# td-kwj-zp2023/webgpu-msm-bls12-377

Measured on AMD Instinct MI355X. Metric: ms per 2^20 BLS12-377 G1 MSM, lower is better.
Workload: dtype u32 (29-bit limbs, 64-bit accumulate)

## Files before the change

### webgpu-msm-bls12-377_amd/csrc/capi.hip

```cpp
#include <hip/hip_runtime.h>
#include <stdlib.h>
#include <string.h>

#include <algorithm>
#include <new>

#include "context.hpp"
#include "host_tail.hpp"
#include "sequencer.hpp"
#include "import_host.hpp"
#include "validate_host.hpp"

using namespace msm377;

#define HIP_TRY(ctx, call)                                                  \
  do {                                                                      \
    if (!eng::hip_ok((ctx), (int)(call), #call)) return MSM377_EHIP;        \
  } while (0)


extern "C" {

const char* msm377_version(void) { return "msm377 0.1 gfx950"; }

const char* msm377_strerror(int code) {
  switch (code) {
    case MSM377_OK: return "ok";
    case MSM377_EINVAL: return "invalid argument";
    case MSM377_EHIP: return "HIP runtime error";
    case MSM377_ESCALAR: return "scalar out of range for the signed window recode";
    case MSM377_ENOMEM: return "out of memory";
    case MSM377_ESTATE: return "call sequence error";
    case MSM377_EGLVRANGE: return "scalar outside the GLV range";
    case MSM377_EEXCEPTIONAL: return "exceptional case of the twisted Edwards law while combining partial records";
    case MSM377_EPOINT: return "an input point failed a requested check (canonical / on the curve / in the subgroup)";
    default: return "unknown error";
  }
}

int msm377_ctx_create(int device, uint64_t max_points, msm377_ctx** out) {
  if (!out || max_points == 0 || max_points > (1ull << 30)) return MSM377_EINVAL;
  *out = nullptr;
  int count = 0;
  if (hipGetDeviceCount(&count) != hipSuccess || device < 0 || device >= count) return MSM377_EHIP;
  msm377_ctx* ctx = new (std::nothrow) msm377_ctx();
  if (!ctx) return MSM377_ENOMEM;
  ctx->device = device;
  ctx->cap = max_points;
  if (const char* e = getenv("MSM377_GLV")) ctx->glv_mode = atoi(e);
  if (const char* e = getenv("MSM377_G1_FORM")) ctx->g1_form = atoi(e) != 0;
  if (const char* e = getenv("MSM377_CONV_WAVE_PRIO")) ctx->conv_wave_prio = atoi(e) != 0;
  if (const char* e = getenv("MSM377_AFF_PREWAKE_US")) ctx->aff_prewake_us = atoll(e);
  if (const char* e = getenv("MSM377_UPLOAD_CHUNKS")) ctx->upload_chunks = (uint32_t)std::min(std::max(atoi(e), 2), 7);
  if (const char* e = getenv("MSM377_UPLOAD_SPLIT")) ctx->upload_split_pct = (uint32_t)std::min(std::max(atoi(e), 5), 90);
  if (const char* e = getenv("MSM377_UPLOAD_CHUNK_MIN")) ctx->upload_chunk_min = strtoull(e, nullptr, 10);
  if (const char* e = getenv("MSM377_TAIL_THREADS")) ctx->tail_threads = std::min(std::max(atoi(e), 1), TailPool::WORKERS + 1);
  if (const char* e = getenv("MSM377_TAIL_WAIT_MS")) ctx->tail_pool.wait_limit_ns = (int64_t)std::max(atoi(e), 1) * 1000000ll;
  if (const char* e = getenv("MSM377_TAIL_SPIN_US")) ctx->tail_spin_us = atoll(e);
  if (const char* e = getenv("MSM377_TAIL_TRACE")) ctx->tail_trace = atoi(e) != 0;
  if (const char* e = getenv("MSM377_TAIL_NUMA")) ctx->tail_pool.numa_local = atoi(e) != 0;
  if (const char* e = getenv("MSM377_TE_AFFINE_MSM")) ctx->te_affine_msm = atoi(e) != 0;
  if (const char* e = getenv("MSM377_NARROW_MAX")) ctx->narrow_max_points = strtoull(e, nullptr, 10);
  if (const char* e = getenv("MSM377_PRECOMP_BITS")) ctx->precomp_bits = atoi(e) == (int)WIDE_BITS ? (int)WIDE_BITS : MSM377_WINDOW_BITS;
  if (const char* e = getenv("MSM377_AFFINE_MIN")) ctx->affine_min_points = strtoull(e, nullptr, 10);
  if (const char* e = getenv("MSM377_SEG_PLAIN")) ctx->seg_plain = std::min(std::max(atoi(e), (int)SEG_MIN), (int)SEG_MAX);
  if (const char* e = getenv("MSM377_SEG_GLV")) ctx->seg_glv = std::min(std::max(atoi(e), (int)SEG_MIN), (int)SEG_MAX);
  if (const char* e = getenv("MSM377_ZERO_COPY_OUT")) ctx->zc_out = atoi(e);
  if (const char* e = getenv("MSM377_NARROW_SEG")) ctx->narrow_seg = (uint32_t)std::min(std::max(atoi(e), (int)NARROW_SEG), (int)SEG_BINS - 1);
  if (const char* e = getenv("MSM377_NARROW_QUAD_ITEMS")) ctx->narrow_quad_items = strtoull(e, nullptr, 10);
  if (const char* e = getenv("MSM377_COOP_THREADS")) ctx->coop_threads = (uint32_t)atoi(e);
  if (const char* e = getenv("MSM377_NARROW_TAIL_FROM")) ctx->narrow_tail_from = (uint32_t)std::min(std::max(atoi(e), 1), (int)TREE_LEVELS);
  if (const char* e = getenv("MSM377_TAIL_LDS")) ctx->tail_lds = atoi(e) != 0;
  if (const char* e = getenv("MSM377_EVEN_WINDOWS")) ctx->even_windows = atoi(e) != 0;
  if (const char* e = getenv("MSM377_TWIN_BATCH")) ctx->twin_batches = atoi(e) != 0;
  if (const char* e = getenv("MSM377_BASE_CHECKS")) ctx->base_checks = check_flags_normal((uint32_t)strtoul(e, nullptr, 0));
  if (const char* e = getenv("MSM377_TAIL_FROM")) ctx->tail_from = (uint32_t)std::min(std::max(atoi(e), 1), (int)TREE_LEVELS);
  const uint64_t cap = max_points;
  int prio_least = 0, prio_greatest = 0;
  bool ok = hipSetDevice(device) == hipSuccess;
  if (ok && hipDeviceGetStreamPriorityRange(&prio_least, &prio_greatest) != hipSuccess) prio_least = prio_greatest = 0;
  ok = ok && hipStreamCreateWithPriority(&ctx->stream, hipStreamNonBlocking, prio_greatest) == hipSuccess &&
            hipStreamCreateWithPriority(&ctx->stream2, hipStreamNonBlocking, prio_least) == hipSuccess &&
            hipEventCreateWithFlags(&ctx->bases_ready, hipEventDisableTiming) == hipSuccess;
  auto dalloc = [&](void** p, size_t bytes) { ok = ok && hipMalloc(p, bytes) == hipSuccess; };
  dalloc((void**)&ctx->d_raw_points, cap * 96);
  dalloc((void**)&ctx->d_raw_scalars, cap * 32);
  dalloc((void**)&ctx->d_bases, 2 * cap * G1_REC_WORDS * 4);
  const uint64_t wcap = std::max<uint64_t>((uint64_t)MSM377_NUM_WINDOWS * cap, (uint64_t)NARROW_EVEN_WINDOWS * std::min<uint64_t>(cap, SMALL_SORT_MAX));
  dalloc((void**)&ctx->d_digits, wcap * 2);
  dalloc((void**)&ctx->d_range_counts, (size_t)NRANGE * MAX_SORT_BLOCKS * 4);
  dalloc((void**)&ctx->d_region_base, (size_t)MSM377_NUM_WINDOWS * (NRANGE + 1) * 4);
  dalloc((void**)&ctx->d_sort_temp, cap * MSM377_NUM_WINDOWS * sizeof(SortElem));
  dalloc((void**)&ctx->d_row_ptr, (size_t)MSM377_NUM_WINDOWS * RP * 4);
  dalloc((void**)&ctx->d_val_idx, wcap * 4);
  dalloc((void**)&ctx->d_buckets, (size_t)MSM377_NUM_WINDOWS * BKT_WORDS * NB * 4);
  dalloc((void**)&ctx->d_partials, (size_t)2 * SLOT_WORDS * 4);
  const uint64_t extra_items = std::max<uint64_t>((uint64_t)MSM377_NUM_WINDOWS * cap / SEG_MIN, (uint64_t)NARROW_EVEN_WINDOWS * std::min<uint64_t>(cap, SMALL_SORT_MAX) / NARROW_SEG) + 2;
  dalloc((void**)&ctx->d_work, ((size_t)MSM377_NUM_WINDOWS * NB + extra_items) * sizeof(WorkItem));
  dalloc((void**)&ctx->d_work_meta, (size_t)META_BLOCK_WORDS * 4);
  dalloc((void**)&ctx->d_row_ovf_base, (size_t)MSM377_NUM_WINDOWS * NB * 4);
  dalloc((void**)&ctx->d_split_rows, (size_t)MSM377_NUM_WINDOWS * NB * 4);
  dalloc((void**)&ctx->d_ovf, (size_t)extra_items * BKT_WORDS * 4);
  const size_t aff_blocks = (size_t)affine_blocks(cap) + 1;
  dalloc((void**)&ctx->d_aff_count, 64);
  ok = ok && hipMemset(ctx->d_aff_count, 0, 64) == hipSuccess;
  dalloc((void**)&ctx->d_aff_stash, (size_t)affine_blocks(cap) * AFF_BLOCK_POINTS * AFF_STASH_WORDS * 4);
  dalloc((void**)&ctx->d_aff_trees, aff_blocks * 2 * AFF_THREADS * 13 * 4);
  const unsigned host_flags = hipHostMallocMapped | hipHostMallocCoherent;
  ok = ok && hipHostMalloc((void**)&ctx->h_aff_prod, aff_blocks * 48, host_flags) == hipSuccess &&
       hipHostMalloc((void**)&ctx->h_aff_inv, aff_blocks * 48, host_flags) == hipSuccess &&
       hipHostMalloc((void**)&ctx->h_aff_flag, 64, host_flags) == hipSuccess &&
       hipHostGetDevicePointer((void**)&ctx->dm_aff_prod, ctx->h_aff_prod, 0) == hipSuccess &&
       hipHostGetDevicePointer((void**)&ctx->dm_aff_inv, ctx->h_aff_inv, 0) == hipSuccess &&
       hipHostGetDevicePointer((void**)&ctx->dm_aff_flag, ctx->h_aff_flag, 0) == hipSuccess &&
       hipEventCreateWithFlags(&ctx->aff_up_done, hipEventDisableTiming) == hipSuccess;
  if (ok) ctx->aff_scratch.resize(aff_blocks);
  dalloc((void**)&ctx->d_err, 4 * sizeof(int));
  ok = ok && hipHostMalloc((void**)&ctx->h_partials, (size_t)2 * SLOT_WORDS * 4, host_flags) == hipSuccess &&
       hipHostGetDevicePointer((void**)&ctx->dm_partials, ctx->h_partials, 0) == hipSuccess &&
       hipHostMalloc((void**)&ctx->h_out_flag, 64, host_flags) == hipSuccess &&
       hipHostGetDevicePointer((void**)&ctx->dm_out_flag, ctx->h_out_flag, 0) == hipSuccess;
  if (ok) memset(ctx->h_out_flag, 0, 64);
  dalloc((void**)&ctx->d_out_count, 64);
  ok = ok && hipMemset(ctx->d_out_count, 0, 64) == hipSuccess;
  ok = ok && hipHostMalloc((void**)&ctx->h_err, 2 * sizeof(int)) == hipSuccess;
  for (int k = 0; ok && k < 2; k++) ok = ok && hipEventCreateWithFlags(&ctx->done_ev[k], hipEventDisableTiming) == hipSuccess;
  for (int s = 0; ok && s < MSM377_NUM_STAGES; s++)
    for (int k = 0; k < 2; k++) ok = ok && hipEventCreate(&ctx->ev[s][k]) == hipSuccess;
  if (!ok) {
    msm377_ctx_destroy(ctx);
    return MSM377_ENOMEM;
  }
  *out = ctx;
  return MSM377_OK;
}

void msm377_ctx_destroy(msm377_ctx* ctx) {
  if (!ctx) return;
  ctx->tail_pool.shutdown();
  (void)hipSetDevice(ctx->device);
  if (ctx->stream) (void)hipStreamSynchronize(ctx->stream);
  if (ctx->stream2) (void)hipStreamSynchronize(ctx->stream2);
  if (ctx->twin) {
    eng::twin_return(ctx);
    msm377_ctx_destroy(ctx->twin);
    ctx->twin = nullptr;
  }
  void* bufs[] = {ctx->d_raw_points, ctx->d_raw_scalars, ctx->d_bases, ctx->d_digits, ctx->d_range_counts, ctx->d_region_base, ctx->d_sort_temp,
// ... 312 lines not shown
```

### webgpu-msm-bls12-377_amd/csrc/common.hpp

```cpp
#pragma once
#include <stdint.h>

#include "../../include/msm377.h"

namespace msm377 {

constexpr uint32_t NB = 32768;
constexpr uint32_t NBIN = NB + 1;
constexpr uint32_t RP = NBIN + 1;
constexpr uint32_t PT_WORDS = 52;
constexpr uint32_t BKT_WORDS = 64;
constexpr uint32_t MAX_SORT_BLOCKS = 256;
constexpr uint32_t TREE_LEVELS = 15;
constexpr uint32_t SEG_MIN = 16;
constexpr uint32_t SEG_MAX = 128;
constexpr uint32_t SEG_BINS = SEG_MAX + 1;
constexpr int ERR_SCALAR = 1, ERR_GLV_RANGE = 2, ERR_NARROW_RANGE = 128;
constexpr int ERR_SHORT_WIDTH = 256;
constexpr int ERR_TE_EXCEPTIONAL = MSM377_FB_ACCUMULATE, ERR_TE_MERGE = MSM377_FB_MERGE, ERR_TE_TREE = MSM377_FB_TREE, ERR_TE_CONVERT = MSM377_FB_CONVERT;
constexpr int ERR_TE_ANY = ERR_TE_EXCEPTIONAL | ERR_TE_MERGE | ERR_TE_TREE | ERR_TE_CONVERT;
constexpr uint32_t NARROW_LOG = 11;
constexpr uint32_t NARROW_SEG = 8;
constexpr uint32_t NARROW_EVEN_WINDOWS = 22, NARROW_EVEN_SIGNED = 11, NARROW_EVEN_BITS = NARROW_LOG + 1;
static_assert(NARROW_EVEN_SIGNED * NARROW_EVEN_BITS + (NARROW_EVEN_WINDOWS - NARROW_EVEN_SIGNED) * NARROW_LOG == 253, "the windows cover a 253-bit scalar");
constexpr uint32_t MAX_WINDOW_SLOTS = NARROW_EVEN_WINDOWS > MSM377_NUM_WINDOWS ? NARROW_EVEN_WINDOWS : MSM377_NUM_WINDOWS;

constexpr uint32_t short_windows(uint32_t bits, uint32_t L) { return bits / (L + 1) + 1; }
static_assert(short_windows(253, 15) == MSM377_NUM_WINDOWS && short_windows(253, NARROW_LOG) == NARROW_EVEN_WINDOWS, "at full width: the window counts of the main and the narrow path");

constexpr uint32_t NRANGE = 256;
constexpr uint32_t KRANGE = NB / NRANGE;
constexpr uint32_t KEY_TRACKED = 0x80000000u;
constexpr uint32_t KEY_UNSIGNED = 0x40000000u;
constexpr uint32_t SMALL_SORT_MAX = 1u << 16;
constexpr uint32_t SMALL_BINS_MAX = (1u << 12) + 1;
struct SortElem {
  uint32_t idx_sign;
  uint32_t key;
};

struct WorkItem {
  uint32_t row;
  uint32_t seg;
};
constexpr uint32_t META_BLOCK_WORDS = 2 * SEG_BINS + 4 + MSM377_NUM_WINDOWS;
constexpr size_t SLOT_WORDS = (size_t)MAX_WINDOW_SLOTS * MSM377_G1_PARTIAL_POINTS * MSM377_G1_POINT_WORDS;

constexpr uint32_t AFF_THREADS = 256, AFF_K = 8, AFF_BLOCK_POINTS = AFF_THREADS * AFF_K;
constexpr uint32_t AFF_STASH_WORDS = 52;
inline uint32_t affine_blocks(uint64_t n) { return (uint32_t)((n + AFF_BLOCK_POINTS - 1) / AFF_BLOCK_POINTS); }

constexpr uint32_t ACC_FLAG_WORD = 4;
constexpr uint32_t EVEN_FROM = 13;
constexpr uint32_t even_offset(uint32_t w) { return 16 * w - (w > EVEN_FROM ? w - EVEN_FROM : 0u); }
static_assert(even_offset(13) == 208 && even_offset(14) == 223 && even_offset(15) == 238 && even_offset(16) == 253, "13 x 16 + 3 x 15 = 253 bits");
constexpr uint32_t WIDE_BITS = MSM377_WIDE_WINDOW_BITS;
constexpr uint32_t WIDE_LOG = 19;
constexpr uint32_t WIDE_WINDOWS = 13;
constexpr uint32_t WIDE_FULL = 6;
constexpr uint32_t wide_width(uint32_t w) { return w < WIDE_FULL ? WIDE_BITS : WIDE_BITS - 1; }
constexpr uint32_t wide_offset(uint32_t w) { return w <= WIDE_FULL ? WIDE_BITS * w : WIDE_BITS * WIDE_FULL + (WIDE_BITS - 1) * (w - WIDE_FULL); }
static_assert(wide_offset(WIDE_WINDOWS - 1) == 234 && wide_offset(WIDE_WINDOWS - 1) + wide_width(WIDE_WINDOWS - 1) == 253, "the windows cover a 253-bit scalar");
constexpr uint32_t WIDE_NRANGE = 4096;
constexpr uint32_t WIDE_POINTS = WIDE_LOG + 1;
static_assert((1u << WIDE_LOG) == WIDE_NRANGE * KRANGE, "ranges of KRANGE keys cover the wide bucket set");
static_assert((1u << WIDE_LOG) <= MSM377_NUM_WINDOWS * NB, "the wide bucket set fits the main path's bucket, row and work-list buffers");
static_assert(WIDE_POINTS * 1 <= MAX_WINDOW_SLOTS * MSM377_G1_PARTIAL_POINTS, "the wide window record fits a partial-record slot");

constexpr uint32_t G1_REC_WORDS = 32;
constexpr uint32_t GLV_WINDOWS = MSM377_GLV_WINDOWS;

}
```

### webgpu-msm-bls12-377_amd/csrc/context.hpp

```cpp
#pragma once
#include <hip/hip_runtime.h>

#include <functional>
#include <string>
#include <vector>

#include "common.hpp"
#include "fp64_host.hpp"
#include "tail_pool.hpp"

using msm377::SortElem;
using msm377::WorkItem;
using msm377::TailPool;
using msm377::Fp64;
using msm377::MAX_WINDOW_SLOTS;
using msm377::NARROW_SEG;

struct ResidentBases {
  uint64_t n = 0;
  int form = 0;
  uint32_t* bases = nullptr;
  uint32_t* table = nullptr;
  uint64_t cap = 0;
  uint32_t windows = 0;
// ... 7 lines not shown
};

struct WideBuffers {
  uint32_t* digits = nullptr;
  SortElem* temp = nullptr;
  uint32_t* counts = nullptr;
  uint64_t cap = 0;
  bool ensure(uint64_t n);
  void release() {
    for (void* p : {(void*)digits, (void*)temp, (void*)counts}) (void)hipFree(p);
    *this = WideBuffers();
  }
};

struct msm377_ctx {
  int device = 0;
  hipStream_t stream = nullptr;
  hipStream_t stream2 = nullptr;
  hipEvent_t bases_ready = nullptr;
  uint64_t cap = 0;
  std::string err;
  uint32_t* d_raw_points = nullptr;
  uint32_t* d_raw_scalars = nullptr;
  uint32_t* d_bases = nullptr;
  uint16_t* d_digits = nullptr;
  uint32_t* d_range_counts = nullptr;
  uint32_t* d_region_base = nullptr;
  SortElem* d_sort_temp = nullptr;
  uint32_t* d_row_ptr = nullptr;
  uint32_t* d_val_idx = nullptr;
  uint32_t* d_buckets = nullptr;
  uint32_t* d_buckets_snap = nullptr;
  uint32_t* d_partials = nullptr;
  WorkItem* d_work = nullptr;
  uint32_t* d_work_meta = nullptr;
  uint32_t* d_row_ovf_base = nullptr;
  uint32_t* d_split_rows = nullptr;
  uint32_t* d_ovf = nullptr;
  uint32_t point_form = MSM377_POINTS_WIRE, scalar_form = MSM377_SCALARS_WIRE;
  uint8_t* d_native = nullptr;
  uint32_t* d_inf_mask = nullptr;
  hipEvent_t import_done = nullptr;
  ResidentBases resident;
  WideBuffers wide;
  int precomp_bits = MSM377_WINDOW_BITS;
  uint32_t* d_aff_stash = nullptr;
  uint32_t* d_aff_trees = nullptr;
  uint32_t* h_aff_prod = nullptr;
  uint32_t* h_aff_inv = nullptr;
  uint32_t* h_aff_flag = nullptr;
  uint32_t *dm_aff_prod = nullptr, *dm_aff_inv = nullptr, *dm_aff_flag = nullptr;
  uint32_t* d_aff_count = nullptr;
  hipEvent_t aff_up_done = nullptr;
  std::vector<Fp64::El> aff_scratch;
  bool te_affine_msm = true;
  uint64_t affine_min_points = 1ull << 20;
  int* d_err = nullptr;
  uint32_t* h_partials = nullptr;
  int* h_err = nullptr;
  hipEvent_t done_ev[2] = {};
  uint8_t* h_stage = nullptr;
  hipStream_t copy_stream[8] = {};
  uint64_t last_n = 0;
  uint32_t last_wc = 0;
  uint32_t last_geom_windows = 0, last_geom_log = 0;
  int last_form = -1;
  bool capture = false;
  int zc_out = 1;
  bool zc_active = false;
  uint32_t out_seq = 0;
  uint32_t* h_out_flag = nullptr;
  uint32_t* dm_out_flag = nullptr;
  uint32_t* dm_partials = nullptr;
  uint32_t* d_out_count = nullptr;
  int timing = 0;
  uint32_t coop_threads = 131072;
  uint32_t narrow_tail_from = 4;
  uint32_t narrow_seg = 0;
  uint64_t narrow_quad_items = 100000;
  uint32_t tail_from = 7;
  int glv_mode = 0;
  int g1_form = 1;
  bool last_glv = false;
  uint32_t seg_plain = 0, seg_glv = 0;
  hipEvent_t ev[MSM377_NUM_STAGES][2] = {};
  uint64_t upload_chunk_min = 1ull << 18;
  uint32_t upload_chunks = 4;
  uint32_t upload_split_pct = 30;
  std::function<int()> before_accumulate;
  TailPool tail_pool;
  int tail_threads = 6;
  int64_t aff_prewake_us = 600;
  uint32_t conv_wave_prio = 1;
  int64_t tail_spin_us = 1000;
  bool tail_trace = false;
  double stage_ms[MSM377_NUM_STAGES] = {};
  int last_products = 0;
  uint64_t narrow_max_points = 1ull << 16;
  bool tail_lds = true;
  bool even_windows = true;
  bool ed_equal_windows_once = false;
  uint32_t acc_seq = 0;
  msm377_ctx* twin = nullptr;
  bool twin_batches = true;
  bool twin_failed = false;
  uint32_t base_checks = 0;
  msm377_check_report last_check = {0, 0, 0, 0, UINT64_MAX, 0, 0};
  uint64_t fallback_count = 0;
  uint32_t fallback_mask = 0;
};
```

### webgpu-msm-bls12-377_amd/csrc/kernels/sort.hpp

```cpp
#pragma once
#include "../curves.hpp"
#include "decompose.hpp"

namespace msm377 {
namespace {



template <class F>
__device__ __forceinline__ void for_each_digit(const uint16_t* __restrict__ dg, uint64_t beg, uint64_t end, uint32_t tid, uint32_t nthreads, F f) {
  uint64_t head = beg;
  while (head < end && (((uintptr_t)(dg + head)) & 15)) head++;
  for (uint64_t i = beg + tid; i < head; i += nthreads) f(i, (uint32_t)dg[i]);
  const uint64_t groups = (end - head) / 8;
  const uint4* v = reinterpret_cast<const uint4*>(dg + head);
  for (uint64_t g = tid; g < groups; g += nthreads) {
    const uint4 q = v[g];
    const uint32_t w[4] = {q.x, q.y, q.z, q.w};
#pragma unroll
    for (int k = 0; k < 4; k++) {
      f(head + g * 8 + 2 * k, w[k] & 0xffffu);
      f(head + g * 8 + 2 * k + 1, w[k] >> 16);
    }
  }
  for (uint64_t i = head + groups * 8 + tid; i < end; i += nthreads) f(i, (uint32_t)dg[i]);
}

template <bool UNS = false>
__global__ void __launch_bounds__(1024) k_range_count(const uint16_t* __restrict__ digits, uint32_t* __restrict__ counts ,
                                                      uint64_t n, uint32_t chunks, uint64_t per_chunk, const uint32_t* __restrict__ key_max) {
  __shared__ uint32_t cnt[NRANGE];
  const uint32_t c = blockIdx.x, ws = blockIdx.y, tid = threadIdx.x;
  const uint32_t shift = win_shift(key_max[ws]);
  const bool uns = UNS && (key_max[ws] & KEY_UNSIGNED) != 0;
  if (tid < NRANGE) cnt[tid] = 0;
  __syncthreads();
  const uint64_t beg = (uint64_t)c * per_chunk;
  const uint64_t end = (beg + per_chunk < n) ? beg + per_chunk : n;
  for_each_digit(digits + (size_t)ws * n, beg, end, tid, 1024, [&](uint64_t, uint32_t biased) {
    uint32_t key, sign;
    digit_key(biased, uns, key, sign);
    atomicAdd(&cnt[key_range(key, shift)], 1u);
  });
  __syncthreads();
  if (tid < NRANGE) counts[((size_t)ws * NRANGE + tid) * chunks + c] = cnt[tid];
}

__global__ void __launch_bounds__(NRANGE) k_range_scan(uint32_t* __restrict__ counts, uint32_t* __restrict__ region_base, uint32_t chunks) {
  __shared__ uint32_t part[NRANGE];
  const uint32_t ws = blockIdx.x, r = threadIdx.x;
  uint32_t* cr = counts + ((size_t)ws * NRANGE + r) * chunks;
  uint32_t tot = 0;
  for (uint32_t c = 0; c < chunks; c++) tot += cr[c];
  part[r] = tot;
  __syncthreads();
  for (uint32_t off = 1; off < NRANGE; off <<= 1) {
    const uint32_t v = r >= off ? part[r - off] : 0u;
    __syncthreads();
    part[r] += v;
    __syncthreads();
  }
  const uint32_t base = part[r] - tot;
  region_base[ws * (NRANGE + 1) + r] = base;
  if (r == NRANGE - 1) region_base[ws * (NRANGE + 1) + NRANGE] = part[r];
  uint32_t run = base;
  for (uint32_t c = 0; c < chunks; c++) {
    const uint32_t v = cr[c];
    cr[c] = run;
    run += v;
  }
}

constexpr uint32_t PT_TILE = 8192;
template <bool UNS = false>
__global__ void __launch_bounds__(1024) k_partition_staged(const uint16_t* __restrict__ digits, const uint32_t* __restrict__ counts,
                                                           SortElem* __restrict__ temp, uint64_t n, uint32_t chunks, uint64_t per_chunk,
                                                           const uint32_t* __restrict__ key_max) {
  __shared__ uint32_t cur[NRANGE];
  __shared__ uint32_t cnt[NRANGE];
  __shared__ uint32_t toff[NRANGE];
  __shared__ uint32_t gdelta[NRANGE];
  __shared__ uint32_t wsum[NRANGE / 64];
  __shared__ SortElem stage[PT_TILE];
  const uint32_t c = blockIdx.x, ws = blockIdx.y, tid = threadIdx.x;
  const uint32_t shift = win_shift(key_max[ws]);
  const bool uns = UNS && (key_max[ws] & KEY_UNSIGNED) != 0;
  if (tid < NRANGE) {
    cur[tid] = counts[((size_t)ws * NRANGE + tid) * chunks + c];
    cnt[tid] = 0;
  }
  __syncthreads();
  const uint64_t beg = (uint64_t)c * per_chunk;
  const uint64_t end = (beg + per_chunk < n) ? beg + per_chunk : n;
  const uint16_t* dg = digits + (size_t)ws * n;
  SortElem* out = temp + (size_t)ws * n;
  for (uint64_t tile0 = beg; tile0 < end; tile0 += PT_TILE) {
    const uint64_t i0 = tile0 + (uint64_t)tid * 8;
    uint32_t d[8];
    uint32_t valid = 0;
    if (i0 + 8 <= end && (((uintptr_t)(dg + i0)) & 15) == 0) {
      const uint4 q = *reinterpret_cast<const uint4*>(dg + i0);
      const uint32_t w[4] = {q.x, q.y, q.z, q.w};
#pragma unroll
      for (int k = 0; k < 4; k++) {
        d[2 * k] = w[k] & 0xffffu;
        d[2 * k + 1] = w[k] >> 16;
      }
      valid = 0xffu;
    } else {
#pragma unroll
      for (int j = 0; j < 8; j++) {
        d[j] = 0;
        if (i0 + j < end) {
          d[j] = dg[i0 + j];
          valid |= 1u << j;
        }
      }
    }
    uint32_t key[8], sign[8], rg[8], rk[8];
#pragma unroll
    for (int j = 0; j < 8; j++) {
      digit_key(d[j], uns, key[j], sign[j]);
      rg[j] = key_range(key[j], shift);
      rk[j] = 0;
      if ((valid >> j) & 1u) rk[j] = atomicAdd(&cnt[rg[j]], 1u);
    }
    __syncthreads();
    uint32_t mine = 0, incl = 0;
    if (tid < NRANGE) {
      mine = cnt[tid];
      incl = mine;
#pragma unroll
      for (int off = 1; off < 64; off <<= 1) {
        const uint32_t v = __shfl_up((int)incl, off, 64);
        if ((tid & 63) >= (uint32_t)off) incl += v;
      }
      if ((tid & 63) == 63) wsum[tid >> 6] = incl;
    }
    __syncthreads();
    if (tid < NRANGE) {
      uint32_t before = 0;
      for (uint32_t w = 0; w < (tid >> 6); w++) before += wsum[w];
      const uint32_t excl = before + incl - mine;
      toff[tid] = excl;
      gdelta[tid] = cur[tid] - excl;
      cur[tid] += mine;
      cnt[tid] = 0;
    }
    __syncthreads();
#pragma unroll
    for (int j = 0; j < 8; j++)
      if ((valid >> j) & 1u) stage[toff[rg[j]] + rk[j]] = SortElem{(uint32_t)(i0 + j) | (sign[j] << 31), key[j]};
    __syncthreads();
    const uint32_t tile_len = (uint32_t)((end - tile0 < PT_TILE) ? end - tile0 : PT_TILE);
    for (uint32_t p = tid; p < tile_len; p += 1024) {
      const SortElem e = stage[p];
      out[gdelta[key_range(e.key, shift)] + p] = e;
    }
    __syncthreads();
  }
}

constexpr uint32_t LS_CACHE = 6144;
constexpr uint32_t LS_REG = LS_CACHE / 256;
__global__ void __launch_bounds__(256) k_local_sort_lds(const SortElem* __restrict__ temp, const uint32_t* __restrict__ region_base,
                                                        uint32_t* __restrict__ row_ptr, uint32_t* __restrict__ val_idx, uint64_t n,
                                                        const uint32_t* __restrict__ key_max, uint32_t NR, uint32_t NBK) {
  constexpr uint32_t NBINS = KRANGE + 1;
  static_assert(NBINS <= 256, "one bin per thread");
  __shared__ uint32_t bins[NBINS];
  __shared__ uint32_t part[256];
  __shared__ uint32_t sorted[LS_CACHE];
  const uint32_t RPW = NBK + 2;
  const uint32_t r = blockIdx.x, ws = blockIdx.y, tid = threadIdx.x;
  const uint32_t shift = key_max ? win_shift(key_max[ws]) : 0u;
  const uint32_t KR = KRANGE >> shift;
  const uint32_t lo = r * KR;
  const bool last = shift == 0 && r == NR - 1;
  const uint32_t nb = KR + (last ? 1u : 0u);
  const uint32_t rbeg = region_base[ws * (NR + 1) + r], rend = region_base[ws * (NR + 1) + r + 1];
  const uint32_t len = rend - rbeg;
  const bool cached = len <= LS_CACHE;
  const SortElem* in = temp + (size_t)ws * n + rbeg;
  if (tid < NBINS) bins[tid] = 0;
  __syncthreads();
  SortElem e[LS_REG];
  if (cached) {
#pragma unroll
    for (uint32_t u = 0; u < LS_REG; u++) {
      const uint32_t i = u * 256 + tid;
      e[u].key = lo;
      e[u].idx_sign = 0;
      if (i < len) e[u] = in[i];
    }
#pragma unroll
    for (uint32_t u = 0; u < LS_REG; u++)
      if (u * 256 + tid < len) atomicAdd(&bins[e[u].key - lo], 1u);
  } else {
    for (uint32_t i0 = 0; i0 < len; i0 += 2048) {
      SortElem f[8];
#pragma unroll
      for (int u = 0; u < 8; u++) {
        const uint32_t i = i0 + u * 256 + tid;
        f[u].key = lo;
        f[u].idx_sign = 0;
        if (i < len) f[u] = in[i];
      }
#pragma unroll
      for (int u = 0; u < 8; u++)
        if (i0 + u * 256 + tid < len) atomicAdd(&bins[f[u].key - lo], 1u);
    }
  }
  __syncthreads();
  const uint32_t own = tid < nb ? bins[tid] : 0u;
  part[tid] = own;
  __syncthreads();
  for (uint32_t off = 1; off < 256; off <<= 1) {
    const uint32_t v = tid >= off ? part[tid - off] : 0u;
    __syncthreads();
    part[tid] += v;
    __syncthreads();
  }
  uint32_t* rp = row_ptr + (size_t)ws * RPW + lo;
  const uint32_t start = rbeg + part[tid] - own;
  __syncthreads();
  if (tid < nb) {
    bins[tid] = start;
    rp[tid] = start;
  }
  if (tid == 0 && last) rp[nb] = rend;
  if (shift) {
    const uint32_t covered = NR * KR, total = region_base[ws * (NR + 1) + NR];
    const uint32_t per_block = (RPW - covered + NR - 1) / NR;
    uint32_t* rp_w = row_ptr + (size_t)ws * RPW;
    for (uint32_t j = tid; j < per_block; j += 256) {
      const uint32_t idx = covered + r * per_block + j;
      if (idx < RPW) rp_w[idx] = total;
    }
  }
  __syncthreads();
  uint32_t* vi = val_idx + (size_t)ws * n;
  if (cached) {
#pragma unroll
    for (uint32_t u = 0; u < LS_REG; u++)
      if (u * 256 + tid < len) sorted[atomicAdd(&bins[e[u].key - lo], 1u) - rbeg] = e[u].idx_sign;
    __syncthreads();
    for (uint32_t i = tid; i < len; i += 256) vi[rbeg + i] = sorted[i];
  } else {
    for (uint32_t i0 = 0; i0 < len; i0 += 2048) {
      SortElem f[8];
#pragma unroll
      for (int u = 0; u < 8; u++) {
        const uint32_t i = i0 + u * 256 + tid;
        f[u].key = lo;
        f[u].idx_sign = 0;
        if (i < len) f[u] = in[i];
      }
#pragma unroll
      for (int u = 0; u < 8; u++) {
        const uint32_t i = i0 + u * 256 + tid;
        if (i < len) vi[atomicAdd(&bins[f[u].key - lo], 1u)] = f[u].idx_sign;
      }
    }
  }
}

__global__ void __launch_bounds__(1024) k_small_sort(const uint16_t* __restrict__ digits, uint32_t* __restrict__ row_ptr, uint32_t* __restrict__ val_idx,
                                                     uint32_t n, uint32_t L) {
  __shared__ uint32_t bins[SMALL_BINS_MAX + 1];
  __shared__ uint32_t part[1024];
  const uint32_t ws = blockIdx.x, tid = threadIdx.x;
  const uint32_t half = 1u << L, nbins = half + 1;
  const uint16_t* dg = digits + (size_t)ws * n;
  for (uint32_t b = tid; b <= nbins; b += 1024) bins[b] = 0;
  __syncthreads();
  for (uint32_t i = tid; i < n; i += 1024) {
    const int d = (int)dg[i] - (int)half;
    atomicAdd(&bins[d < 0 ? -d : d], 1u);
  }
  __syncthreads();
  const uint32_t per = (nbins + 1023) / 1024;
  uint32_t local = 0;
  for (uint32_t k = 0; k < per; k++) {
    const uint32_t b = tid * per + k;
    if (b < nbins) local += bins[b];
  }
  part[tid] = local;
  __syncthreads();
  for (uint32_t off = 1; off < 1024; off <<= 1) {
    const uint32_t v = tid >= off ? part[tid - off] : 0u;
    __syncthreads();
    part[tid] += v;
    __syncthreads();
  }
  uint32_t run = part[tid] - local;
  uint32_t* rp = row_ptr + (size_t)ws * (half + 2);
  for (uint32_t k = 0; k < per; k++) {
    const uint32_t b = tid * per + k;
    if (b < nbins) {
      const uint32_t cnt = bins[b];
      bins[b] = run;
      rp[b] = run;
      run += cnt;
    }
  }
  if (tid == 0) rp[nbins] = n;
  __syncthreads();
  uint32_t* vi = val_idx + (size_t)ws * n;
  for (uint32_t i = tid; i < n; i += 1024) {
    const int d = (int)dg[i] - (int)half;
    vi[atomicAdd(&bins[d < 0 ? -d : d], 1u)] = i | (d < 0 ? 0x80000000u : 0u);
  }
}

}
}
```

### webgpu-msm-bls12-377_amd/csrc/sequencer.hip

```cpp
#include "sequencer.hpp"

#include <hip/hip_runtime.h>
#include <string.h>

#include <algorithm>
#include <atomic>
#include <chrono>
#include <functional>
#include <thread>
#include <type_traits>
#include <vector>

#include "context.hpp"
#include "host_tail.hpp"
#include "validate_host.hpp"
#include "kernels/accumulate.hpp"
#include "kernels/convert.hpp"
#include "kernels/decompose.hpp"
#include "kernels/generate.hpp"
#include "kernels/reduce.hpp"
#include "kernels/sort.hpp"
#include "kernels/validate.hpp"
#include "kernels/import.hpp"
#include "kernels/wide.hpp"
// ... 160 lines not shown
    return MSM377_EHIP;
  }
  {
    const int inv_rc = invert_block_products_mt(ctx, 0, nblk);
    ctx->tail_pool.disarm();
    if (inv_rc) return inv_rc;
  }
  hipLaunchKernelGGL(k_affine_down, dim3(nblk), dim3(AFF_THREADS), 0, ctx->stream2, n, ctx->d_aff_stash, ctx->d_aff_trees, ctx->dm_aff_inv, d_records_out, ctx->conv_wave_prio);
  HIP_TRY(ctx, hipGetLastError());
  if (ctx->timing == 1) (void)hipEventRecord(ctx->ev[MSM377_STAGE_CONVERT][1], ctx->stream2);
  HIP_TRY(ctx, hipEventRecord(ctx->bases_ready, ctx->stream2));
  return MSM377_OK;
}

uint32_t auto_seg(const msm377_ctx* ctx, uint64_t entries, bool glv) {
  const uint32_t forced = glv ? ctx->seg_glv : ctx->seg_plain;
  if (forced) return forced;
  const uint64_t s = ((entries >> 18) + 7) & ~7ull;
  return (uint32_t)std::min<uint64_t>(std::max<uint64_t>(s, SEG_MIN), SEG_MAX);
}


struct Phase {
  bool clear_err = true;
  bool front = true;
  bool into = false;
  bool back = true;
  bool zc_out = false;
  uint64_t base_first = 0;
  const uint32_t* table = nullptr;
  uint64_t table_stride = 0;
  uint32_t cbits = MSM377_WINDOW_BITS;
  uint32_t bucket_log = MSM377_WINDOW_BITS - 1;
  bool wide = false;
  bool even = false;
  const uint32_t* bases_override = nullptr;
  uint32_t short_bytes = 0, short_bits = 0;
};

void launch_decompose_short(hipStream_t st, const void* d_scalars, uint16_t* digits, uint64_t n, uint32_t sbytes, uint32_t bits, uint32_t L, uint32_t W, uint32_t bias,
                            uint32_t top_bias, int* d_err, uint32_t* top_key_max) {
  const dim3 grid((unsigned)((n + 255) / 256)), block(256);
  const uint8_t* sc = (const uint8_t*)d_scalars;
  switch (sbytes) {
    case 4: hipLaunchKernelGGL(k_decompose_short<4>, grid, block, 0, st, sc, digits, n, bits, L, W, bias, top_bias, d_err, top_key_max); break;
    case 8: hipLaunchKernelGGL(k_decompose_short<8>, grid, block, 0, st, sc, digits, n, bits, L, W, bias, top_bias, d_err, top_key_max); break;
    case 16: hipLaunchKernelGGL(k_decompose_short<16>, grid, block, 0, st, sc, digits, n, bits, L, W, bias, top_bias, d_err, top_key_max); break;
    default: hipLaunchKernelGGL(k_decompose_short<32>, grid, block, 0, st, sc, digits, n, bits, L, W, bias, top_bias, d_err, top_key_max); break;
  }
}

template <class CV, class BP = CV>
int enqueue_windows(msm377_ctx* ctx, const uint32_t* d_scalars, uint64_t n_scalars, uint32_t wb, uint32_t wc, int slot, bool glv = false,
                    const Phase& ph = Phase()) {
  const uint64_t n = glv ? 2 * n_scalars : n_scalars;
  hipStream_t st = ctx->stream;
  int* d_err = ctx->d_err + slot;
  uint32_t* d_partials = ctx->d_partials + (size_t)slot * SLOT_WORDS;
  if (ph.clear_err && !ph.front) hipLaunchKernelGGL(k_clear_words, dim3(1), dim3(256), 0, st, (uint32_t*)d_err, 1u, (uint32_t*)nullptr, 0u);
  ctx->zc_active = ph.zc_out && ph.back && ctx->zc_out && slot == 0 && !ph.table;
  if (ctx->zc_active) ctx->out_seq++;
  const uint32_t L = ph.bucket_log, NB = 1u << L;
  const bool wide = ph.wide;
  const bool narrow = !wide && ph.cbits != MSM377_WINDOW_BITS;
  const uint64_t entries = (wide ? (uint64_t)WIDE_WINDOWS : (uint64_t)wc) * n;
  static_assert((uint64_t)NARROW_EVEN_WINDOWS * SMALL_SORT_MAX / NARROW_SEG + NARROW_EVEN_WINDOWS * (1u << NARROW_LOG) <= (uint64_t)MSM377_NUM_WINDOWS * 32768,
                "narrow work items fit the work-item buffer");
  const uint32_t SEG = (narrow && !ctx->seg_plain) ? (ctx->narrow_seg ? ctx->narrow_seg : (n > 8192 ? 16u : 12u)) : auto_seg(ctx, entries, glv);
  uint16_t* digits = ctx->d_digits;
  uint32_t* range_counts = ctx->d_range_counts;
  uint32_t* region_base = ctx->d_region_base;
  SortElem* sort_temp = ctx->d_sort_temp;
  uint32_t* row_ptr = ctx->d_row_ptr;
  uint32_t* val_idx = ctx->d_val_idx;
  uint32_t* buckets = ctx->d_buckets;
  uint32_t* row_ovf_base = ctx->d_row_ovf_base;
  uint32_t* split_rows = ctx->d_split_rows;
  WorkItem* work = ctx->d_work;
  uint32_t* ovf = ctx->d_ovf;
  const uint32_t* records = ctx->resident.valid() ? ctx->resident.bases : ctx->d_bases;
  const uint32_t* bases = ph.table ? ph.table : ph.bases_override ? ph.bases_override : records + ph.base_first * BP::REC_WORDS;
  uint32_t* meta_block = ctx->d_work_meta;
  uint32_t* key_max = meta_block + (2 * SEG_BINS + 4);
  if (ph.front) {
    hipLaunchKernelGGL(k_clear_words, dim3(1), dim3(256), 0, st, meta_block, META_BLOCK_WORDS, (uint32_t*)d_err, ph.clear_err ? 1u : 0u);
    uint32_t* top_key_max = (!glv && !ph.even && wb + wc == MSM377_NUM_WINDOWS) ? key_max + (wc - 1) : nullptr;
    const uint64_t max_items = (uint64_t)wc * NB + entries / SEG;
    const bool quad_acc = std::is_same<BP, CV>::value && std::is_same<CV, TeDev>::value && narrow && !ph.table && max_items <= ctx->narrow_quad_items;
    {
      StageTimer t(ctx, MSM377_STAGE_DECOMPOSE, st);
      if (ph.short_bytes)
        launch_decompose_short(st, d_scalars, digits, n, ph.short_bytes, ph.short_bits, L, wc, narrow ? NB : 32768u, narrow ? NB : 0u, d_err, narrow ? nullptr : key_max + (wc - 1));
      else if (wide)
        hipLaunchKernelGGL(k_decompose_wide, dim3((unsigned)((n + 255) / 256)), dim3(256), 0, st, d_scalars, ctx->wide.digits, n, d_err);
      else if (narrow)
        hipLaunchKernelGGL(k_decompose_geom, dim3((unsigned)((n + 255) / 256)), dim3(256), 0, st, d_scalars, digits, n, L, NARROW_EVEN_SIGNED, wc, 1u << L, d_err);
      else if (glv)
        hipLaunchKernelGGL(k_decompose_glv, dim3((unsigned)((n_scalars + 255) / 256)), dim3(256), 0, st, d_scalars, digits, n_scalars, wb, wc, d_err);
      else
        hipLaunchKernelGGL(k_decompose, dim3((unsigned)((n + 255) / 256)), dim3(256), 0, st, d_scalars, digits, n, wb, wc, d_err, top_key_max, ph.even ? 1u : 0u);
      HIP_TRY(ctx, hipGetLastError());
    }

    if (wide) {
      StageTimer t(ctx, MSM377_STAGE_SORT, st);
      uint32_t* wc = ctx->wide.counts;
      hipLaunchKernelGGL(k_wide_count, dim3(WS_CHUNKS, WIDE_WINDOWS), dim3(1024), 0, st, (const uint32_t*)ctx->wide.digits, wc, n);
      hipLaunchKernelGGL(k_wide_sums, dim3(WIDE_NRANGE / 256, WIDE_WINDOWS), dim3(256), 0, st, wc);
      hipLaunchKernelGGL(k_wide_scan, dim3(1), dim3(1024), 0, st, wc, region_base);
      hipLaunchKernelGGL(k_wide_offsets1, dim3(WIDE_WINDOWS), dim3(WS_COARSE), 0, st, wc, n);
      hipLaunchKernelGGL(k_wide_part1, dim3(WS_CHUNKS, WIDE_WINDOWS), dim3(1024), 0, st, (const uint32_t*)ctx->wide.digits, (const uint32_t*)wc, sort_temp, n, (uint32_t)ph.table_stride);
      hipLaunchKernelGGL(k_wide_part2, dim3(WS_COARSE, WIDE_WINDOWS), dim3(1024), 0, st, (const SortElem*)sort_temp, (const uint32_t*)wc, ctx->wide.temp);
      hipLaunchKernelGGL(k_local_sort_lds, dim3(WIDE_NRANGE, 1), dim3(256), 0, st, (const SortElem*)ctx->wide.temp, region_base, row_ptr, val_idx, entries,
                         (const uint32_t*)nullptr, WIDE_NRANGE, NB);
      HIP_TRY(ctx, hipGetLastError());
    } else if (narrow) {
      StageTimer t(ctx, MSM377_STAGE_SORT, st);
      hipLaunchKernelGGL(k_small_sort, dim3(wc), dim3(1024), 0, st, digits, row_ptr, val_idx, (uint32_t)n, L);
      HIP_TRY(ctx, hipGetLastError());
    } else {
      StageTimer t(ctx, MSM377_STAGE_SORT, st);
      uint32_t chunks = MAX_SORT_BLOCKS / wc;
      const uint64_t want = (n + 4095) / 4096;
      if (chunks > want) chunks = (uint32_t)(want ? want : 1);
      const uint64_t per_chunk = (n + chunks - 1) / chunks;
      if (ph.short_bytes)
        hipLaunchKernelGGL(k_range_count<true>, dim3(chunks, wc), dim3(1024), 0, st, digits, range_counts, n, chunks, per_chunk, key_max);
      else
        hipLaunchKernelGGL(k_range_count<false>, dim3(chunks, wc), dim3(1024), 0, st, digits, range_counts, n, chunks, per_chunk, key_max);
      HIP_TRY(ctx, hipGetLastError());
      hipLaunchKernelGGL(k_range_scan, dim3(wc), dim3(NRANGE), 0, st, range_counts, region_base, chunks);
      HIP_TRY(ctx, hipGetLastError());
      if (ph.short_bytes)
        hipLaunchKernelGGL(k_partition_staged<true>, dim3(chunks, wc), dim3(1024), 0, st, digits, range_counts, sort_temp, n, chunks, per_chunk, key_max);
      else
        hipLaunchKernelGGL(k_partition_staged<false>, dim3(chunks, wc), dim3(1024), 0, st, digits, range_counts, sort_temp, n, chunks, per_chunk, key_max);
      HIP_TRY(ctx, hipGetLastError());
      hipLaunchKernelGGL(k_local_sort_lds, dim3(NRANGE, wc), dim3(256), 0, st, sort_temp, region_base, row_ptr, val_idx, n, key_max, NRANGE, NB);
      HIP_TRY(ctx, hipGetLastError());
    }

    {
      StageTimer t(ctx, MSM377_STAGE_ACCUMULATE, st);
      const uint32_t rows = wc * NB;
      uint32_t* meta = meta_block;
      uint32_t* work_hist = meta;
      uint32_t* cursor = meta + SEG_BINS;
      uint32_t* total = meta + 2 * SEG_BINS;
      uint32_t* counters = meta + 2 * SEG_BINS + 1;
      hipLaunchKernelGGL(k_work_hist, dim3((rows + 1023) / 1024), dim3(1024), 0, st, row_ptr, L, rows, SEG, work_hist, row_ovf_base, counters, split_rows);
      HIP_TRY(ctx, hipGetLastError());
      hipLaunchKernelGGL(k_work_scatter, dim3((rows + 1023) / 1024), dim3(1024), 0, st, row_ptr, L, rows, SEG, (const uint32_t*)work_hist, cursor, total, work);
      HIP_TRY(ctx, hipGetLastError());
      if (ctx->before_accumulate) {
        std::function<int()> f;
        f.swap(ctx->before_accumulate);
        const int hook_rc = f();
        if (hook_rc) return hook_rc;
      }
      HIP_TRY(ctx, hipStreamWaitEvent(st, ctx->bases_ready, 0));
      ctx->last_products = BP::MADD_PRODUCTS;
      {
        StageTimer tk(ctx, MSM377_STAGE_ACC_KERNEL, st);
        const dim3 grid((unsigned)((max_items + 255) / 256));
        bool launched = false;
        if constexpr (std::is_same<BP, CV>::value && std::is_same<CV, TeDev>::value) {
          if (quad_acc) {
            hipLaunchKernelGGL(k_accumulate_quad<CV>, dim3((unsigned)((4 * max_items + 255) / 256)), dim3(256), 0, st, row_ptr, val_idx, bases, buckets, n, work, total,
                               row_ovf_base, ovf, SEG, d_err, ctx->d_err + 2, ph.into ? 1u : 0u, L);
            launched = true;
          }
        }
        if (launched) {
        } else if constexpr (!std::is_same<BP, CV>::value)
          hipLaunchKernelGGL((k_accumulate<CV, 2, BP>), grid, dim3(256), 0, st, row_ptr, val_idx, bases, buckets, n, work, total, row_ovf_base, ovf, SEG, d_err,
                             ctx->d_err + 2, ph.into ? 1u : 0u, ph.table_stride, L);
        else
          hipLaunchKernelGGL((k_accumulate<CV, 2>), grid, dim3(256), 0, st, row_ptr, val_idx, bases, buckets, n, work, total, row_ovf_base, ovf, SEG, d_err,
                             ctx->d_err + 2, ph.into ? 1u : 0u, ph.table_stride, L);
      }
      HIP_TRY(ctx, hipGetLastError());
      ctx->acc_seq++;
      static_assert(CV::HAS_QUAD, "every curve policy has the quad-cooperative addition");
      if (ph.short_bytes) {
        hipLaunchKernelGGL(k_fold_long_rows<CV>, dim3(FOLD_BLOCKS), dim3(FOLD_THREADS), 0, st, row_ptr, row_ovf_base, ovf, SEG, d_err, L, wc - 1);
        HIP_TRY(ctx, hipGetLastError());
      }
      hipLaunchKernelGGL(k_merge_split_rows_quad<CV>, dim3(std::min<uint32_t>((rows + 63) / 64, 1024u)), dim3(256), 0, st, row_ptr, buckets, counters, split_rows, row_ovf_base, ovf, SEG, d_err, L,
                         ctx->dm_out_flag + ACC_FLAG_WORD, ctx->acc_seq);
      HIP_TRY(ctx, hipGetLastError());
    }
  }
  if (!ph.back) return MSM377_OK;
  if (ctx->capture) {
    HIP_TRY(ctx, hipMemcpyAsync(ctx->d_buckets_snap, buckets, (size_t)wc * CV::BKT_WORDS * NB * 4, hipMemcpyDeviceToDevice, st));
  }
  const uint32_t wc_out = ph.table ? 1u : wc;
  const uint32_t pp = wide ? WIDE_POINTS : (uint32_t)MSM377_G1_PARTIAL_POINTS;
  {
    StageTimer t(ctx, MSM377_STAGE_REDUCE, st);
    if (ph.table) {
      for (uint32_t m = wc; m > 1;) {
        const uint32_t half = (m + 1) / 2, count = m - half;
        hipLaunchKernelGGL(k_fold_windows<CV>, dim3(count * NB / 256), dim3(256), 0, st, buckets, L, half, count, d_err);
        HIP_TRY(ctx, hipGetLastError());
        m = half;
      }
    }
    const uint32_t levels = L;
    uint32_t coop_from = 0;
    for (coop_from = 0; coop_from < levels && 4ull * (coop_from + 1) * (NB >> (coop_from + 1)) * wc_out > ctx->coop_threads; coop_from++) {
      }
    const uint32_t tail_from = CV::HAS_QUAD ? std::min(wide ? levels - 8 : narrow ? ctx->narrow_tail_from : ctx->tail_from, levels) : levels;
    for (uint32_t r = 0; r < tail_from; r++) {
      const uint32_t ops = (r + 1) * (NB >> (r + 1));
      bool done = false;
      if constexpr (CV::HAS_QUAD) {
        if (r >= coop_from) {
          hipLaunchKernelGGL(k_tree_step_quad<CV>, dim3((4 * ops + 255) / 256, wc_out), dim3(256), 0, st, buckets, L, r, ops, d_err);
          done = true;
        }
      }
      if (!done) hipLaunchKernelGGL(k_tree_step<CV>, dim3((ops + 255) / 256, wc_out), dim3(256), 0, st, buckets, L, r, ops, d_err);
      HIP_TRY(ctx, hipGetLastError());
    }
    if constexpr (CV::HAS_QUAD) {
      if (tail_from < levels) {
        const size_t lds_bytes = (size_t)(NB >> tail_from) * CV::PT_WORDS * 4;
        if (ctx->tail_lds && lds_bytes > 64 * 1024 && lds_bytes <= TAIL_LDS_BYTES_MAX)
          HIP_TRY(ctx, hipFuncSetAttribute(reinterpret_cast<const void*>(&k_reduce_tail_lds<CV>), hipFuncAttributeMaxDynamicSharedMemorySize, (int)TAIL_LDS_BYTES_MAX));
        if (ctx->tail_lds && lds_bytes <= TAIL_LDS_BYTES_MAX)
          hipLaunchKernelGGL(k_reduce_tail_lds<CV>, dim3(tail_from + 1, wc_out), dim3(TAIL_THREADS), lds_bytes, st, buckets, L, tail_from, d_err);
        else
// ... 1342 lines not shown
```

### webgpu-msm-bls12-377_amd/csrc/te377.hpp

```cpp
#pragma once
#include "ed_ext.hpp"
#include "field29.hpp"

namespace msm377 {

template <class F_, class K_>
struct TeLazy {
  using F = F_;
  using El = typename F::El;
  using K = K_;
  struct ABase {
    El ymx, ypx, kt;
  };
  struct PBase {
    El ymx, ypx, kt, z2;
  };
  struct Ext {
    El x, y, t, z;
  };
  static MSM_HD Ext identity() {
    Ext r;
    r.x = F::zero();
    r.y = F::one();
    r.t = F::zero();
    r.z = F::one();
    return r;
  }
  static MSM_HD bool is_zero_mod_p(const El& a) { return F::is_zero(a) || F::eq(a, F::from_const(K::MOD)); }
  static MSM_HD bool is_bad(const Ext& p) { return is_zero_mod_p(p.z); }

  static MSM_HD Ext madd(const Ext& p, const PBase& q, bool neg) {
    const El a = F::mul_lz(F::add_kp_sub(p.y, K::KP2, p.x), F::select(neg, q.ypx, q.ymx));
    const El b = F::mul_lz(F::add_lz(p.y, p.x), F::select(neg, q.ymx, q.ypx));
    const El c = F::mul_lz(F::select(neg, F::kp_sub(K::KP2, q.kt), q.kt), p.t);
    const El d = F::mul_lz(p.z, q.z2);
    return finish(a, b, c, d);
  }
  static MSM_HD Ext madd_affine(const Ext& p, const ABase& q, bool neg) {
    const El a = F::mul_lz(F::add_kp_sub(p.y, K::KP2, p.x), F::select(neg, q.ypx, q.ymx));
    const El b = F::mul_lz(F::add_lz(p.y, p.x), F::select(neg, q.ymx, q.ypx));
    const El c = F::mul_lz(F::select(neg, F::kp_sub(K::KP2, q.kt), q.kt), p.t);
    return finish(a, b, c, F::add_lz(p.z, p.z));
  }
  static MSM_HD Ext add(const Ext& p, const Ext& q) {
    const El a = F::mul_lz(F::norm(F::add_kp_sub(p.y, K::KP2, p.x)), F::norm(F::add_kp_sub(q.y, K::KP2, q.x)));
    const El b = F::mul_lz(F::norm(F::add_lz(p.y, p.x)), F::norm(F::add_lz(q.y, q.x)));
    const El c = F::mul_lz(F::mul_lz(p.t, q.t), F::from_const(K::TE_2D));
    const El d = F::mul_lz(p.z, q.z);
    return finish(a, b, c, F::add_lz(d, d));
  }
  static MSM_HD Ext finish(const El& a, const El& b, const El& c, const El& d) {
    const El e = F::norm(F::add_kp_sub(b, K::KP2, a));
    const El f = F::norm(F::add_kp_sub(d, K::KP2, c));
    const El g = F::norm(F::add_lz(d, c));
    const El h = F::add_lz(b, a);
    Ext r;
    r.x = F::mul_lz(e, f);
    r.y = F::mul_lz(h, g);
    r.t = F::mul_lz(h, e);
    r.z = F::mul_lz(f, g);
    return r;
  }
};

using EdLazy = TeLazy<Fq, EdConsts>;

struct Te377 : TeLazy<Fp, G1Consts> {
  using F = Fp;
  using El = Fp::El;
  using K = G1Consts;

  static MSM_HD PBase from_wire(const uint32_t* x12, const uint32_t* y12, bool phi) {
    const El xr = F::template from_words<12>(x12), yr = F::template from_words<12>(y12);
    const El u = F::add(F::mul(xr, F::from_const(phi ? K::TE_SBR : K::TE_SR)), F::from_const(K::TE_S));
    const El v = F::mul(yr, F::from_const(K::TE_SR));
    const El cu = F::add(F::mul(xr, F::from_const(phi ? K::TE_CSBR : K::TE_CSR)), F::from_const(K::TE_CS));
    const El up = F::add(u, F::one());
    const El X = F::mul(cu, up), Z = F::mul(v, up);
    const El T = F::sub(X, F::dbl(cu)), Y = F::sub(Z, F::dbl(v));
    PBase b;
    b.ymx = F::sub(Y, X);
    b.ypx = F::add(Y, X);
    b.kt = F::mul(T, F::from_const(K::TE_2D));
    b.z2 = F::dbl(Z);
    return b;
  }

  static MSM_HD Ext from_base(const PBase& q, bool neg) {
    Ext r;
    const El x2 = F::sub(q.ypx, q.ymx), t2 = F::mul(q.kt, F::from_const(K::TE_INV_D));
    r.x = F::cneg(x2, neg);
    r.y = F::add(q.ypx, q.ymx);
    r.t = F::cneg(t2, neg);
    r.z = q.z2;
    return r;
  }
  static MSM_HD Ext from_base_affine(const ABase& q, bool neg) {
    Ext r;
    const El x2 = F::sub(q.ypx, q.ymx), t2 = F::mul(q.kt, F::from_const(K::TE_INV_D));
    r.x = F::cneg(x2, neg);
    r.y = F::add(q.ypx, q.ymx);
    r.t = F::cneg(t2, neg);
    r.z = F::dbl(F::one());
    return r;
  }

  static MSM_HD ABase affine_from_wire(const uint32_t* x12, const uint32_t* y12, bool& bad) {
    const El xr = F::template from_words<12>(x12), yr = F::template from_words<12>(y12);
    const El u = F::add(F::mul(xr, F::from_const(K::TE_SR)), F::from_const(K::TE_S));
    const El v = F::mul(yr, F::from_const(K::TE_SR));
    const El cu = F::add(F::mul(xr, F::from_const(K::TE_CSR)), F::from_const(K::TE_CS));
// ... 16 lines not shown
```

Measured before the change: 2.446.

## Fuse bucket work histogram into local sort kernel and fast-path zero check

The per-row segment-length histogram, overflow-base assignment and split-row list are now computed inside k_local_sort_lds while the row bounds are still in registers. This removes the separate k_work_hist pass over row_ptr for large non-narrow inputs, with a size threshold that can be set from the environment. The sort kernel gains extra LDS atomics, global atomics and a second block barrier. Separately, is_zero_mod_p returns early when the lowest limb rules out both zero and p, so the full comparison runs only when that limb matches.

```diff
diff --git a/webgpu-msm-bls12-377_amd/csrc/capi.hip b/webgpu-msm-bls12-377_amd/csrc/capi.hip
--- a/webgpu-msm-bls12-377_amd/csrc/capi.hip
+++ b/webgpu-msm-bls12-377_amd/csrc/capi.hip
@@ -64,6 +64,7 @@
   if (const char* e = getenv("MSM377_PRECOMP_BITS")) ctx->precomp_bits = atoi(e) == (int)WIDE_BITS ? (int)WIDE_BITS : MSM377_WINDOW_BITS;
   if (const char* e = getenv("MSM377_AFFINE_MIN")) ctx->affine_min_points = strtoull(e, nullptr, 10);
   if (const char* e = getenv("MSM377_SEG_PLAIN")) ctx->seg_plain = std::min(std::max(atoi(e), (int)SEG_MIN), (int)SEG_MAX);
+  if (const char* e = getenv("MSM377_SORT_HIST_MIN")) ctx->sort_hist_min = strtoull(e, nullptr, 10);
   if (const char* e = getenv("MSM377_SEG_GLV")) ctx->seg_glv = std::min(std::max(atoi(e), (int)SEG_MIN), (int)SEG_MAX);
   if (const char* e = getenv("MSM377_ZERO_COPY_OUT")) ctx->zc_out = atoi(e);
   if (const char* e = getenv("MSM377_NARROW_SEG")) ctx->narrow_seg = (uint32_t)std::min(std::max(atoi(e), (int)NARROW_SEG), (int)SEG_BINS - 1);
diff --git a/webgpu-msm-bls12-377_amd/csrc/common.hpp b/webgpu-msm-bls12-377_amd/csrc/common.hpp
--- a/webgpu-msm-bls12-377_amd/csrc/common.hpp
+++ b/webgpu-msm-bls12-377_amd/csrc/common.hpp
@@ -43,6 +43,7 @@
   uint32_t row;
   uint32_t seg;
 };
+constexpr uint64_t SORT_HIST_MIN_DEFAULT = 1ull << 19;
 constexpr uint32_t META_BLOCK_WORDS = 2 * SEG_BINS + 4 + MSM377_NUM_WINDOWS;
 constexpr size_t SLOT_WORDS = (size_t)MAX_WINDOW_SLOTS * MSM377_G1_PARTIAL_POINTS * MSM377_G1_POINT_WORDS;
 
diff --git a/webgpu-msm-bls12-377_amd/csrc/context.hpp b/webgpu-msm-bls12-377_amd/csrc/context.hpp
--- a/webgpu-msm-bls12-377_amd/csrc/context.hpp
+++ b/webgpu-msm-bls12-377_amd/csrc/context.hpp
@@ -113,6 +113,7 @@
   int glv_mode = 0;
   int g1_form = 1;
   bool last_glv = false;
+  uint64_t sort_hist_min = msm377::SORT_HIST_MIN_DEFAULT;
   uint32_t seg_plain = 0, seg_glv = 0;
   hipEvent_t ev[MSM377_NUM_STAGES][2] = {};
   uint64_t upload_chunk_min = 1ull << 18;
diff --git a/webgpu-msm-bls12-377_amd/csrc/kernels/sort.hpp b/webgpu-msm-bls12-377_amd/csrc/kernels/sort.hpp
--- a/webgpu-msm-bls12-377_amd/csrc/kernels/sort.hpp
+++ b/webgpu-msm-bls12-377_amd/csrc/kernels/sort.hpp
@@ -1,5 +1,6 @@
 #pragma once
 #include "../curves.hpp"
+#include "accumulate.hpp"
 #include "decompose.hpp"
 
 namespace msm377 {
@@ -165,12 +166,18 @@
 constexpr uint32_t LS_REG = LS_CACHE / 256;
 __global__ void __launch_bounds__(256) k_local_sort_lds(const SortElem* __restrict__ temp, const uint32_t* __restrict__ region_base,
                                                         uint32_t* __restrict__ row_ptr, uint32_t* __restrict__ val_idx, uint64_t n,
-                                                        const uint32_t* __restrict__ key_max, uint32_t NR, uint32_t NBK) {
+                                                        const uint32_t* __restrict__ key_max, uint32_t NR, uint32_t NBK, uint32_t SEG,
+                                                        uint32_t* __restrict__ work_hist, uint32_t* __restrict__ row_ovf_base,
+                                                        uint32_t* __restrict__ counters ,
+                                                        uint32_t* __restrict__ split_rows) {
   constexpr uint32_t NBINS = KRANGE + 1;
   static_assert(NBINS <= 256, "one bin per thread");
   __shared__ uint32_t bins[NBINS];
   __shared__ uint32_t part[256];
   __shared__ uint32_t sorted[LS_CACHE];
+  __shared__ uint32_t lh[SEG_BINS];
+  __shared__ uint32_t blk[4];
+  static_assert(SEG_BINS <= 256, "one length bin per thread");
   const uint32_t RPW = NBK + 2;
   const uint32_t r = blockIdx.x, ws = blockIdx.y, tid = threadIdx.x;
   const uint32_t shift = key_max ? win_shift(key_max[ws]) : 0u;
@@ -183,6 +190,8 @@
   const bool cached = len <= LS_CACHE;
   const SortElem* in = temp + (size_t)ws * n + rbeg;
   if (tid < NBINS) bins[tid] = 0;
+  if (tid < SEG_BINS) lh[tid] = 0;
+  if (tid < 2) blk[tid] = 0;
   __syncthreads();
   SortElem e[LS_REG];
   if (cached) {
@@ -229,6 +238,17 @@
     rp[tid] = start;
   }
   if (tid == 0 && last) rp[nb] = rend;
+  RowSplit sp = {1, 0, 0};
+  uint32_t my_split = 0, my_ovf = 0;
+  if (work_hist && tid < nb && lo + tid >= 1) {
+    sp = row_split(own, SEG);
+    atomicAdd(&lh[sp.lastlen], 1u);
+    if (sp.nseg > 1) {
+      atomicAdd(&lh[sp.seglen], sp.nseg - 1);
+      my_split = atomicAdd(&blk[0], 1u);
+      my_ovf = atomicAdd(&blk[1], sp.nseg - 1);
+    }
+  }
   if (shift) {
     const uint32_t covered = NR * KR, total = region_base[ws * (NR + 1) + NR];
     const uint32_t per_block = (RPW - covered + NR - 1) / NR;
@@ -237,8 +257,27 @@
       const uint32_t idx = covered + r * per_block + j;
       if (idx < RPW) rp_w[idx] = total;
     }
-  }
-  __syncthreads();
+    if (work_hist && tid == 0) {
+      const uint32_t first = covered + r * per_block, stop = first + per_block < NBK + 1 ? first + per_block : NBK + 1;
+      if (stop > first) atomicAdd(&lh[0], stop - first);
+    }
+  }
+  __syncthreads();
+  if (work_hist) {
+    if (tid < SEG_BINS && lh[tid]) atomicAdd(&work_hist[tid], lh[tid]);
+    if (blk[0]) {
+      if (tid == 0) {
+        blk[2] = atomicAdd(&counters[0], blk[0]);
+        blk[3] = atomicAdd(&counters[1], blk[1]);
+      }
+      __syncthreads();
+      if (sp.nseg > 1) {
+        const uint32_t row = ws * NBK + lo + tid - 1;
+        row_ovf_base[row] = blk[3] + my_ovf;
+        split_rows[blk[2] + my_split] = row;
+      }
+    }
+  }
   uint32_t* vi = val_idx + (size_t)ws * n;
   if (cached) {
 #pragma unroll
diff --git a/webgpu-msm-bls12-377_amd/csrc/sequencer.hip b/webgpu-msm-bls12-377_amd/csrc/sequencer.hip
--- a/webgpu-msm-bls12-377_amd/csrc/sequencer.hip
+++ b/webgpu-msm-bls12-377_amd/csrc/sequencer.hip
@@ -266,6 +266,12 @@
   const uint32_t* bases = ph.table ? ph.table : ph.bases_override ? ph.bases_override : records + ph.base_first * BP::REC_WORDS;
   uint32_t* meta_block = ctx->d_work_meta;
   uint32_t* key_max = meta_block + (2 * SEG_BINS + 4);
+  uint32_t* work_hist = meta_block;
+  const bool sort_hist = !narrow && n >= ctx->sort_hist_min;
+  uint32_t* sort_work_hist = sort_hist ? work_hist : nullptr;
+  uint32_t* cursor = meta_block + SEG_BINS;
+  uint32_t* total = meta_block + 2 * SEG_BINS;
+  uint32_t* counters = meta_block + 2 * SEG_BINS + 1;
   if (ph.front) {
     hipLaunchKernelGGL(k_clear_words, dim3(1), dim3(256), 0, st, meta_block, META_BLOCK_WORDS, (uint32_t*)d_err, ph.clear_err ? 1u : 0u);
     uint32_t* top_key_max = (!glv && !ph.even && wb + wc == MSM377_NUM_WINDOWS) ? key_max + (wc - 1) : nullptr;
@@ -296,7 +302,7 @@
       hipLaunchKernelGGL(k_wide_part1, dim3(WS_CHUNKS, WIDE_WINDOWS), dim3(1024), 0, st, (const uint32_t*)ctx->wide.digits, (const uint32_t*)wc, sort_temp, n, (uint32_t)ph.table_stride);
       hipLaunchKernelGGL(k_wide_part2, dim3(WS_COARSE, WIDE_WINDOWS), dim3(1024), 0, st, (const SortElem*)sort_temp, (const uint32_t*)wc, ctx->wide.temp);
       hipLaunchKernelGGL(k_local_sort_lds, dim3(WIDE_NRANGE, 1), dim3(256), 0, st, (const SortElem*)ctx->wide.temp, region_base, row_ptr, val_idx, entries,
-                         (const uint32_t*)nullptr, WIDE_NRANGE, NB);
+                         (const uint32_t*)nullptr, WIDE_NRANGE, NB, SEG, sort_work_hist, row_ovf_base, counters, split_rows);
       HIP_TRY(ctx, hipGetLastError());
     } else if (narrow) {
       StageTimer t(ctx, MSM377_STAGE_SORT, st);
@@ -320,19 +326,15 @@
       else
         hipLaunchKernelGGL(k_partition_staged<false>, dim3(chunks, wc), dim3(1024), 0, st, digits, range_counts, sort_temp, n, chunks, per_chunk, key_max);
       HIP_TRY(ctx, hipGetLastError());
-      hipLaunchKernelGGL(k_local_sort_lds, dim3(NRANGE, wc), dim3(256), 0, st, sort_temp, region_base, row_ptr, val_idx, n, key_max, NRANGE, NB);
+      hipLaunchKernelGGL(k_local_sort_lds, dim3(NRANGE, wc), dim3(256), 0, st, sort_temp, region_base, row_ptr, val_idx, n, key_max, NRANGE, NB, SEG, sort_work_hist,
+                         row_ovf_base, counters, split_rows);
       HIP_TRY(ctx, hipGetLastError());
     }
 
     {
       StageTimer t(ctx, MSM377_STAGE_ACCUMULATE, st);
       const uint32_t rows = wc * NB;
-      uint32_t* meta = meta_block;
-      uint32_t* work_hist = meta;
-      uint32_t* cursor = meta + SEG_BINS;
-      uint32_t* total = meta + 2 * SEG_BINS;
-      uint32_t* counters = meta + 2 * SEG_BINS + 1;
-      hipLaunchKernelGGL(k_work_hist, dim3((rows + 1023) / 1024), dim3(1024), 0, st, row_ptr, L, rows, SEG, work_hist, row_ovf_base, counters, split_rows);
+      if (!sort_hist) hipLaunchKernelGGL(k_work_hist, dim3((rows + 1023) / 1024), dim3(1024), 0, st, row_ptr, L, rows, SEG, work_hist, row_ovf_base, counters, split_rows);
       HIP_TRY(ctx, hipGetLastError());
       hipLaunchKernelGGL(k_work_scatter, dim3((rows + 1023) / 1024), dim3(1024), 0, st, row_ptr, L, rows, SEG, (const uint32_t*)work_hist, cursor, total, work);
       HIP_TRY(ctx, hipGetLastError());
diff --git a/webgpu-msm-bls12-377_amd/csrc/te377.hpp b/webgpu-msm-bls12-377_amd/csrc/te377.hpp
--- a/webgpu-msm-bls12-377_amd/csrc/te377.hpp
+++ b/webgpu-msm-bls12-377_amd/csrc/te377.hpp
@@ -26,7 +26,10 @@
     r.z = F::one();
     return r;
   }
-  static MSM_HD bool is_zero_mod_p(const El& a) { return F::is_zero(a) || F::eq(a, F::from_const(K::MOD)); }
+  static MSM_HD bool is_zero_mod_p(const El& a) {
+    if (__builtin_expect(a.l[0] != 0u && a.l[0] != K::MOD[0], 1)) return false;
+    return F::is_zero(a) || F::eq(a, F::from_const(K::MOD));
+  }
   static MSM_HD bool is_bad(const Ext& p) { return is_zero_mod_p(p.z); }
 
   static MSM_HD Ext madd(const Ext& p, const PBase& q, bool neg) {
```

Result: faster. 2.417 (median of 5 runs) (-1.2%).
